# OSUrobotics/KinovaGrasping

Measured on AMD Instinct MI355X. Metric: env-steps/sec (whole node) at 4096 envs/GPU, higher is better.
Workload: dtype f32

## Files before the change

### kinovagrasping_amd/csrc/ks_api.hip

```cpp
#include <hip/hip_runtime.h>

#include <algorithm>
#include <cstdio>
#include <cstdlib>
#include <cstring>
#include <type_traits>
#include <map>
#include <string>
#include <vector>

#include "../../include/kinova_sim.h"
#include "ks_env.h"
#include "ks_mlp_tile.h"
#include "ks_select.h"
#include "ks_model_host.h"

using namespace ks;

namespace {

constexpr int WAVE = 64;
thread_local std::string g_create_error;

template <typename T> struct StartPool {
// ... 699 lines not shown
    const long bi = (long)sel * N + i;
    const long len0 = ra.with_replay ? ra.cur_len[bi] : 0;
    const long tt = len0 < H - 1 ? len0 : H - 1;
    const long row = bi * H + tt;
    for (int c = sub; c < S; c += SUBS) {
        const float so = (float)((const R*)ra.sim_obs)[(long)i * S + c];
        const float st = ra.obs[(long)i * S + c];
        const float nx = done ? (float)((const R*)ra.sim_final_obs)[(long)i * S + c] : so;
        if (store) { ra.cur_state[row * S + c] = st; ra.cur_next[row * S + c] = nx; }
        ra.prev_obs[(long)i * S + c] = done ? so : st;
        ra.obs[(long)i * S + c] = so;
    }
    if (store && sub < A) ra.cur_action[row * A + sub] = ra.action[(long)i * A + sub];
    if (sub != 0) return;
    long len1 = len0;
    if (store) {
        ra.cur_reward[row] = rew;
        ra.cur_not_done[row] = done ? 0.0f : 1.0f;
        len1 = tt + 1;
    }
    if (ra.with_replay) {
        if (done && lift && len1 > 0) {
            ra.cur_reward[bi * H + len1 - 1] = rew;
            ra.cur_not_done[bi * H + len1 - 1] = 0.0f;
        }
        ra.cur_len[bi] = len1;
        if (done) {
            const bool keep = len1 - ra.n_steps > 1;
            const long bo = (long)(sel ^ 1) * N + i;
            const bool free_other = __hip_atomic_load(&ra.pub_len[bo], __ATOMIC_ACQUIRE, __HIP_MEMORY_SCOPE_AGENT) == 0;
#ifdef KS_DEBUG_DROPS
            int64_t* dbg = ra.counters + 8 + 4 * 512 + 8;
            if (keep && !free_other) {
                const long long gap = (long long)ra.steps_total[i] - (long long)dbg[i];
                atomicAdd((unsigned long long*)&ra.counters[4], (unsigned long long)gap);
                atomicAdd((unsigned long long*)&ra.counters[5], 1ull);
                atomicMin((long long*)&ra.counters[6], gap);
                __builtin_amdgcn_fence(__ATOMIC_ACQUIRE, "agent");
                if (__hip_atomic_load(&ra.pub_len[bo], __ATOMIC_ACQUIRE, __HIP_MEMORY_SCOPE_AGENT) == 0) atomicAdd((unsigned long long*)&ra.counters[7], 1ull);
            }
            if (keep && free_other) dbg[i] = ra.steps_total[i];
#endif
            if (keep && free_other) {
                __threadfence();
                __hip_atomic_store(&ra.pub_len[bi], (int64_t)len1, __ATOMIC_RELEASE, __HIP_MEMORY_SCOPE_AGENT);
                ra.cur_sel[i] = (uint8_t)(sel ^ 1);
                ra.cur_len[bo] = 0;
                atomicAdd((unsigned long long*)&ra.counters[2], 1ull);
            } else {
                ra.cur_len[bi] = 0;
                if (keep) atomicAdd((unsigned long long*)&ra.counters[3], 1ull);
            }
        }
    }
    if (done) {
        atomicAdd((unsigned long long*)&ra.counters[0], 1ull);
        if (ra.sim_done[i] & 1) atomicAdd((unsigned long long*)&ra.counters[1], 1ull);
    }
    ra.has_prev[i] = !done;
    ra.t[i] = done ? 0 : ra.t[i] + 1;
    __hip_atomic_store(&ra.steps_total[i], ra.steps_total[i] + 1, __ATOMIC_RELAXED, __HIP_MEMORY_SCOPE_AGENT);
    ra.ready[i] = (ra.ready[i] != 0) && !done;
    ra.reward_out[i] = rew;
    ra.done_out[i] = done;
}

constexpr int ROLLOUT_QCAP = 2048, ROLLOUT_Q_STEPS = 16, ROLLOUT_Q_RING = ROLLOUT_Q_STEPS + ROLLOUT_QCAP, ROLLOUT_Q_WORDS = ROLLOUT_Q_RING + ROLLOUT_QCAP;
__global__ void k_rollout_queue_init(int* __restrict__ queue, int n_groups) {
    for (int i = threadIdx.x; i < ROLLOUT_Q_WORDS; i += blockDim.x) {
        int v = 0;
        if (i == 1) v = n_groups;
        if (i >= ROLLOUT_Q_RING && i - ROLLOUT_Q_RING < n_groups) v = (1 << 12) | (i - ROLLOUT_Q_RING + 1);
        queue[i] = v;
    }
}

template <int NT1, int NT2>
__device__ __noinline__ void rollout_policy_wave(const ks_rollout_args* __restrict__ rap, int N, int row_env, KS_LDS float* wblocks) {
    const ks_rollout_args& ra = *rap;
    const int S = krsel::S, A = krsel::A;
    constexpr int NR = 4;
    kmlp::f32x4(*H1)[NR] = (kmlp::f32x4(*)[NR])(float*)wblocks;
    kmlp::f32x4(*H2)[NR] = H1 + NT1 * 4;
    const int lane = threadIdx.x & 63;
    for (;;) {
        const long long ver = uniform64(__hip_atomic_load(ra.actor_ver, __ATOMIC_RELAXED, __HIP_MEMORY_SCOPE_AGENT));
        __builtin_amdgcn_fence(__ATOMIC_ACQUIRE, "agent");
        const float* pw = ra.actor_pub + (ver % 3) * ra.actor_stride;
        kmlp::f32x4 z4 = {0.f, 0.f, 0.f, 0.f};
        const bool mine = kmlp::mlp3_rows_wave<NT1, NT2, true, NR>(lane, (long)row_env, S, ra.h1, ra.h2, A, ra.obs, S, kmlp::x_bytes(N, 0, S, S), pw + ra.off_w1,
                                                                     pw + ra.off_b1, pw + ra.off_w2, pw + ra.off_b2, pw + ra.off_w3, H1, H2, z4);
        float y[4] = {0.f, 0.f, 0.f, 0.f};
        if (mine) policy_squash(ra, z4, pw + ra.off_b3, y);
        __builtin_amdgcn_fence(__ATOMIC_ACQUIRE, "agent");
        const long long ver2 = uniform64(__hip_atomic_load(ra.actor_ver, __ATOMIC_RELAXED, __HIP_MEMORY_SCOPE_AGENT));
        if (ver2 - ver < 2) {
            if (mine) policy_select(ra, N, row_env, y);
            return;
        }
        if (lane == 0 && ra.repeats) atomicAdd((unsigned long long*)ra.repeats, 1ull);
    }
}

#ifdef KS_ROLLOUT_STAMP
#define KS_RS(i) { const long long t1_ = wall_clock64(); if (C::tid() == 0) atomicAdd((unsigned long long*)&rap->counters[4 + i], (unsigned long long)(t1_ - tk)); tk = t1_; }
#else
#define KS_RS(i)
#endif
template <int NT1, int NT2, bool WAVE_SCOPE>
__device__ __forceinline__ void rollout_iter(const Model<float>& m, const Hulls<float>& hu, const Buffers<float>* __restrict__ bdev, int N, int frame_skip,
                                             int iters, int epw, int pair_memory, const ObsOut<float>* __restrict__ out,
                                             const ks_rollout_args* __restrict__ rap, KS_LDS float* blocks, int grp) {
    using T = float;
    using C = Crew<WAVE_SCOPE>;
    const Buffers<T>& b = *bdev;
    const int e = threadIdx.x / LANE_STRIDE;
    const Team<SUBS> team{(int)threadIdx.x % LANE_STRIDE};
    const int env = e < epw ? b.slot_env[grp * epw + e] : -1;
    const bool active = !(team.sub >= SUBS || env < 0);
    const int wave = WAVE_SCOPE ? (int)(threadIdx.x >> 6) : 0;
    const int slot0 = grp * epw + 4 * wave, cepw = WAVE_SCOPE ? (epw - 4 * wave < 4 ? (epw - 4 * wave < 0 ? 0 : epw - 4 * wave) : 4) : epw;
    KS_LDS T* cblocks = blocks + 4 * wave * SCR_TOTAL;
    KS_LDS unsigned* w = (KS_LDS unsigned*)cblocks;
    const auto join = [] {
        if constexpr (!WAVE_SCOPE) __threadfence_block();
        C::sync();
    };
#ifdef KS_ROLLOUT_STAMP
    long long tk = wall_clock64();
#endif
    {
        const int nn = C::tid() & 15;
        const int row_env = nn < cepw ? b.slot_env[slot0 + nn] : -1;
        if (b.ctl->mode != 0) rollout_controller(b.ctl, rap, N, C::tid() < 16 ? row_env : -1);
        else if constexpr (WAVE_SCOPE) rollout_policy_wave<NT1, NT2>(rap, N, row_env, cblocks);
        else rollout_policy<NT1, NT2>(rap, N, row_env, cblocks);
    }
    join();
    KS_RS(0)
    if (active) {
        T hq[4], act[4];
        KS_UNROLL
        for (int i = 0; i < 4; i++) { hq[i] = b.hand_quat[(long)i * N + env]; act[i] = rap->action_t[(long)i * N + env]; }
        int ncon = 0, status = 0;
        ColW<T> snap{b.snap + env, N};
        KS_LDS T* blk = blocks + e * SCR_TOTAL;
        ScratchC<T, KS_LDS T*> scr{blk};
        T* stp = (T*)(blk + SCR_STATE);
        load_state_team<T, SUBS>(b, env, N, stp, team.sub);
        load_env_params(scr, team, b, env, N);
        constexpr int WPL = (NPAIR_MAX + SUBS - 1) / SUBS;
        PairWarm gw[WPL];
        unsigned* pm = b.pairmem + ((long)env * SUBS + team.sub) * (WPL * WARM_WORDS);
        KS_UNROLL
        for (int q = 0; q < WPL; q++) {
            KS_UNROLL
            for (int j = 0; j < WARM_WORDS; j++) gw[q].w[j] = pair_memory ? pm[q * WARM_WORDS + j] : 0u;
        }
        lane_env_step(m, hu, *(LaneState<T>*)stp, hq, act, scr, team, snap, frame_skip, iters, ncon, status, (float*)nullptr, stp + NQ + 2 * NV, gw,
                      []() {});
        if (pair_memory) {
            KS_UNROLL
            for (int q = 0; q < WPL; q++) {
                KS_UNROLL
                for (int j = 0; j < WARM_WORDS; j++) pm[q * WARM_WORDS + j] = gw[q].w[j];
            }
        }
        team.sync();
        store_state_team<T, SUBS>(b, env, N, stp, team.sub);
        if (status) atomicOr(&b.status[env], status);
        if (team.sub == 0) b.ncon[env] = ncon;
    }
    join();
    KS_RS(1)
// ... 1034 lines not shown
    }
    void reset_pass(const Buffers<T>& e, void* obs, hipStream_t s) {
        const int N = cfg.n_envs;
        hipLaunchKernelGGL((k_reset<T, USE_LDS>), dim3(blocks()), dim3(WAVE), 0, s, d_model, e, N, 0);
        hipLaunchKernelGGL((k_rays<T>), dim3((N + RAY_ENVS - 1) / RAY_ENVS, NRAY), dim3(WAVE), 0, s, d_model, e, N, 1);
        hipLaunchKernelGGL((k_obs<T>), dim3(blocks()), dim3(WAVE), 0, s, d_model, e, N, 1, out_record(obs, nullptr, nullptr, nullptr, nullptr));
    }
    int post_reset(void* obs, hipStream_t s) {
        if (b.rayq) HIPCHK(hipMemsetAsync(b.rayq, 0, (4 + 2 * (size_t)n_wg) * sizeof(int32_t), s));
        reset_pass(b, obs, s);
        HIPCHK(hipGetLastError());
        return KS_OK;
    }
    int reset(const int32_t* ids, int n, const void* q0, const void* hq, const int32_t* object_id, const void* mass_friction, void* obs,
              hipStream_t s) override {
        if (int r = need_model("ks_reset")) return r;
        if (n <= 0 || n > cfg.n_envs || !q0 || !hq || (!ids && n != cfg.n_envs)) { error = "ks_reset: bad arguments"; return KS_ERR_INVALID; }
        hipLaunchKernelGGL((k_store_init<T>), dim3((n + 255) / 256), dim3(256), 0, s, b, ids, n, (const T*)q0, (const T*)hq, object_id,
                           (const T*)mass_friction, n_models, cfg.n_envs);
        if (object_id) {
            clear_pool(s);
            clear_ranges(s);
            if (n_models > 1)
                if (int r = regroup(s)) return r;
        }
        return post_reset(obs, s);
    }
    int step(const void* action, void* obs, void* reward, uint8_t* done, void* info, void* final_obs, hipStream_t s) override {
        if (int r = need_model("ks_step")) return r;
        if (!action) { error = "ks_step: action is NULL"; return KS_ERR_INVALID; }
        const int N = cfg.n_envs;
        const bool timed = ev_used < NEV && (step_calls++ % ev_stride) == 0;
        const ObsOut<T> out = out_record(obs, reward, done, info, final_obs);
        const bool capturing = stream_is_capturing(s);
        if (obs_in_step && (capturing || captured_out > 0 || !(out == out_sent && out_valid))) {
            out_valid = !capturing;
            out_sent = out;
            ObsOut<T>* slot = pinned_record(capturing, h_out, (unsigned)h_out_next++, captured_out);
            if (!slot) { error = "ks_step: more captured calls than the context keeps output records for"; return KS_ERR_STATE; }
            *slot = out;
            HIPCHK(hipMemcpyAsync(d_out, slot, sizeof out, hipMemcpyHostToDevice, s));
        }
        if (timed) HIPCHK(hipEventRecord(ev0[ev_used], s));
        hipLaunchKernelGGL(step_kernel(), dim3(n_wg), dim3(WG), step_lds, s, d_model, b, (const Buffers<T>*)d_b, (const T*)action, N, cfg.frame_skip,
                           cfg.solver_iterations, lpw, cfg.contact_tap, (int)rays_in_step, (int)(USE_LDS && cfg.pair_memory), (int)obs_in_step,
                           (const ObsOut<T>*)d_out, ray_pool, n_wg);
        if (timed) { HIPCHK(hipEventRecord(ev1[ev_used], s)); ev_used++; }
        if (!rays_in_step) hipLaunchKernelGGL((k_rays<T>), dim3((N + RAY_ENVS - 1) / RAY_ENVS, NRAY), dim3(WAVE), 0, s, d_model, b, N, 0);
        if (!obs_in_step) hipLaunchKernelGGL((k_obs<T>), dim3(blocks()), dim3(WAVE), 0, s, d_model, b, N, 0, out);
        HIPCHK(hipGetLastError());
        return KS_OK;
    }
    int check_rollout_buffers(int n_iter, const ks_rollout_args* ra) {
        if (!ra || n_iter <= 0 || (ctl_mode == 0 && (!ra->actor_pub || !ra->actor_ver)) || !ra->obs || !ra->prev_obs || !ra->has_prev || !ra->ready || !ra->lifting ||
            !ra->t || !ra->steps_total || !ra->action || !ra->action_t || !ra->reward_out || !ra->done_out || !ra->sim_obs || !ra->sim_reward ||
            !ra->sim_done || !ra->sim_info || !ra->sim_final_obs || !ra->counters) { error = "ks_rollout: NULL argument"; return KS_ERR_INVALID; }
        if (ra->with_replay && (!ra->cur_state || !ra->cur_next || !ra->cur_action || !ra->cur_reward || !ra->cur_not_done || !ra->cur_len ||
                                !ra->cur_sel || !ra->pub_len || ra->horizon <= ra->n_steps)) { error = "ks_rollout: replay buffers"; return KS_ERR_INVALID; }
        return KS_OK;
    }
    int check_rollout_actor(const ks_rollout_args* ra) {
        if (ctl_mode != 0) return KS_OK;
        if ((ra->off_w2 | ra->off_w3 | ra->actor_stride) & 3) { error = "ks_rollout: weight offsets must be multiples of 4 floats"; return KS_ERR_INVALID; }
        if ((ra->h1 | ra->h2) & 3) { error = "ks_rollout: hidden widths must be multiples of 4"; return KS_ERR_INVALID; }
        if ((int64_t)cfg.n_envs * krsel::S * 4 >= (int64_t)kmlp::OOR) { error = "ks_rollout: the observation rows exceed the actor's 32-bit lane offsets"; return KS_ERR_INVALID; }
        return KS_OK;
    }
    int send_rollout_records(const ks_rollout_args* ra, hipStream_t s) {
        const ObsOut<T> out = out_record(ra->sim_obs, ra->sim_reward, ra->sim_done, ra->sim_info, ra->sim_final_obs);
        const bool capturing = stream_is_capturing(s);
        ObsOut<T>* slot = pinned_record(capturing, h_out, (unsigned)h_out_next++, captured_out);
        if (!slot) { error = "ks_rollout: more captured calls than the context keeps output records for"; return KS_ERR_STATE; }
        *slot = out;
        out_valid = false;
        HIPCHK(hipMemcpyAsync(d_out, slot, sizeof out, hipMemcpyHostToDevice, s));
        ks_rollout_args* rslot = pinned_record(capturing, h_ra, h_ra_next++, captured_ra);
        if (!rslot) { error = "ks_rollout: more captured calls than the context keeps argument records for"; return KS_ERR_STATE; }
        *rslot = *ra;
        HIPCHK(hipMemcpyAsync(d_ra, rslot, sizeof *ra, hipMemcpyHostToDevice, s));
        return KS_OK;
    }
    static constexpr int policy_tiles(int h1, int h2) { return (h1 + 15) / 16 + (h2 + 15) / 16; }
    static constexpr size_t policy_lds_bytes(int h1, int h2) { return (size_t)(policy_tiles(h1, h2) * 4 + 4) * 16 * 16 + 16; }
    static constexpr size_t policy_wave_lds_bytes(int h1, int h2) { return (size_t)(policy_tiles(h1, h2) * 4) * 4 * 16; }
    template <int A, int B> struct Tiles { static constexpr int NT1 = A, NT2 = B; };
    template <typename F> int launch_for_widths(const ks_rollout_args* ra, F launch) {
        const int t1 = (ra->h1 + 15) / 16, t2 = (ra->h2 + 15) / 16;
        if (t1 == 16 && t2 == 16) return launch(Tiles<16, 16>{});
        if (t1 == 25 && t2 == 19) return launch(Tiles<25, 19>{});
        if (t1 == 8 && t2 == 8) return launch(Tiles<8, 8>{});
        if (t1 == 4 && t2 == 4) return launch(Tiles<4, 4>{});
        if (ctl_mode != 0) return launch(Tiles<16, 16>{});
        error = "ks_rollout: hidden widths must be 256-256, 400-300, 128-128 or 64-64";
        return KS_ERR_INVALID;
    }
    template <typename K, typename... A> int launch_rollout(K kernel, size_t lds, hipStream_t s, A... args) {
        HIPCHK(hipFuncSetAttribute((const void*)kernel, hipFuncAttributeMaxDynamicSharedMemorySize, (int)lds));
        hipLaunchKernelGGL(kernel, dim3(n_groups < resident_wgs ? n_groups : resident_wgs), dim3(WG), lds, s, args...);
        HIPCHK(hipGetLastError());
        return KS_OK;
    }
    int rollout_exact(int n_iter, const ks_rollout_args* ra, hipStream_t s) {
#ifdef KS_MULTI_GEOM
        (void)n_iter; (void)ra; (void)s;
        error = "ks_rollout: libkinova_sim_mg.so runs fp32 contexts only (the exact mode, precision 64, is in libkinova_sim.so)";
        return KS_ERR_INVALID;
#else
        int r;
        if ((r = check_rollout_buffers(n_iter, ra))) return r;
        if (!cfg.obs_env_major || !cfg.auto_reset) { error = "ks_rollout needs env-major observations and auto_reset"; return KS_ERR_STATE; }
        if ((r = check_rollout_actor(ra))) return r;
        if (ra->budget_ticks != 0) { error = "ks_rollout: a time budget needs the wave form of the rollout kernel (ks_rollout_plan: KS_PLAN_WAVES); fp64 contexts have none"; return KS_ERR_STATE; }
        const size_t ws_offset = (step_lds + 15) / 16 * 16;
        const size_t lds = ws_offset + std::max(policy_lds_bytes(ra->h1, ra->h2), (size_t)F64_RAY_BYTES);
        if (lds > 160 * 1024) { error = "ks_rollout: no LDS for the policy beside this object's hull tables"; return KS_ERR_STATE; }
        if ((r = send_rollout_records(ra, s))) return r;
        return launch_for_widths(ra, [&](auto tiles) {
            using W = decltype(tiles);
            return launch_rollout(k_rollout_f64<W::NT1, W::NT2>, lds, s, d_model, b, (const Buffers<T>*)d_b, cfg.n_envs, cfg.frame_skip, cfg.solver_iterations,
                                  lpw, (const ObsOut<T>*)d_out, (const ks_rollout_args*)d_ra, n_iter, rollout_round_robin ? -n_groups : n_groups,
                                  (int)ws_offset);
        });
#endif
    }
    int rollout(int n_iter, const ks_rollout_args* ra, hipStream_t s) override {
        if (int r = need_model("ks_rollout")) return r;
        if constexpr (sizeof(T) != 4) return rollout_exact(n_iter, ra, s);
        else {
            int r;
            if ((r = check_rollout_buffers(n_iter, ra))) return r;
            if (!obs_in_step || !cfg.obs_env_major || !cfg.auto_reset) { error = "ks_rollout needs the in-kernel observation path, env-major observations and auto_reset"; return KS_ERR_STATE; }
            if ((r = check_rollout_actor(ra))) return r;
            if (policy_lds_bytes(ra->h1, ra->h2) > (size_t)SCR_TOTAL * lpw * sizeof(T)) { error = "ks_rollout: no LDS for the policy"; return KS_ERR_STATE; }
            const int N = cfg.n_envs;
            const bool wave_free = plan_waves() && policy_wave_lds_bytes(ra->h1, ra->h2) <= (size_t)SCR_TOTAL * 4 * sizeof(T);
            if (ra->budget_ticks != 0 && (ra->budget_ticks < 0 || !wave_free)) {
                error = "ks_rollout: a time budget needs the wave form of the rollout kernel (ks_rollout_plan: KS_PLAN_WAVES)";
                return KS_ERR_STATE;
            }
            if ((r = send_rollout_records(ra, s))) return r;
            const bool use_queue = plan_queue();
            if (use_queue) {
                hipLaunchKernelGGL(k_rollout_queue_init, dim3(1), dim3(256), 0, s, d_queue, n_groups);
            }
            if (wave_free && rollout_phase_deal != 0 && n_models == 1 && ra->budget_ticks == 0) {
                if (rollout_phase_deal == 2 && N <= PHASE_ENVS_MAX) hipLaunchKernelGGL(k_slots_by_phase, dim3(1), dim3(PHASE_THREADS), 0, s, (const int64_t*)ra->t, N, n_wg * lpw, b.slot_env);
                else if (lpw <= 16) hipLaunchKernelGGL(k_slots_by_phase_in_groups, dim3((n_groups + 255) / 256), dim3(256), 0, s, (const int64_t*)ra->t, n_groups, lpw, b.slot_env);
            }
            return launch_for_widths(ra, [&](auto tiles) {
                using W = decltype(tiles);
                return launch_rollout(k_rollout<W::NT1, W::NT2>, step_lds, s, d_model, b, (const Buffers<T>*)d_b, N, cfg.frame_skip, cfg.solver_iterations, lpw,
                                      (int)cfg.pair_memory, (const ObsOut<T>*)d_out, (const ks_rollout_args*)d_ra, n_iter,
                                      (use_queue || !rollout_round_robin) ? n_groups : -n_groups, use_queue ? d_queue : (int*)nullptr, (int)wave_free);
            });
        }
    }
    bool plan_queue() const { return rollout_queue && n_groups > resident_wgs && n_groups <= ROLLOUT_QCAP; }
    bool plan_waves() const {
        return rollout_waves && !plan_queue() && n_groups <= resident_wgs && lpw == EPW_MAX && LANE_STRIDE == SUBS &&
               (size_t)(wg_rays_words(4, WAVE) + wg_obs_words(4) + 4) <= (size_t)SCR_TOTAL * 4;
    }
    int rollout_plan(int32_t* mode, int32_t* groups, int32_t* workgroups) override {
        if (int r = need_model("ks_rollout_plan")) return r;
        if constexpr (sizeof(T) != 4) {
            if (mode) *mode = n_groups <= resident_wgs ? KS_PLAN_WORKGROUPS : (rollout_round_robin ? KS_PLAN_ROUND_ROBIN : KS_PLAN_RUNS);
        } else if (mode) *mode = plan_waves() ? KS_PLAN_WAVES : (n_groups <= resident_wgs ? KS_PLAN_WORKGROUPS : (plan_queue() ? KS_PLAN_QUEUE : (rollout_round_robin ? KS_PLAN_ROUND_ROBIN : KS_PLAN_RUNS)));
        if (groups) *groups = n_groups;
// ... 331 lines not shown
```

### kinovagrasping_amd/csrc/ks_mlp_tile.h

```cpp
#pragma once
#include <stdint.h>

#if defined(__HIPCC__)
#include <hip/hip_runtime.h>
#define KS_MLP_HD __host__ __device__
#else
#define KS_MLP_HD
#endif

namespace kmlp {

constexpr int ROWS = 16;
constexpr int KS_IN_MAX = 6;

constexpr uint32_t OOR = 0x7ffffff0u;

KS_MLP_HD inline uint32_t tile_soff(int row0, int k0, int K) { return (uint32_t)(row0 * K + k0) * 4u; }
KS_MLP_HD inline uint32_t quad_off(int nn, int q, int row0, int nrow, int k0, int K) {
    const int row = row0 + nn, k = k0 + 4 * q;
    return (row >= 0 && row < nrow && k + 3 < K) ? (uint32_t)(nn * K + 4 * q) * 4u : OOR;
}
KS_MLP_HD inline int tail_k(int K) { return K & ~3; }
KS_MLP_HD inline uint32_t tail_off(int nn, int row0, int nrow, int K, int j) {
    const int row = row0 + nn;
// ... 113 lines not shown
                    const float fb = ldf(rXb, x_off(row, 16 * s + 4 * q + j, in_a, in_dim, ldb), 0);
                    fa[s][j] = 16 * s + 4 * q + j < in_a ? fa[s][j] : fb;
                }
        }
#pragma unroll
        for (int s = 0; s < KS_IN_MAX; s++) bx[s] = f32x4{fa[s][0], fa[s][1], fa[s][2], fa[s][3]};
    }
    Tile<NT1, !VEC> a2, b2t;
    {
        Tile<KS_IN_MAX, true> a1, b1t;
        a1.issue(rW1, rB1, nn, q, 16 * wave, h1, in_dim);
        a2.issue(rW2, rB2, nn, q, 16 * wave, h2, h1);
        auto tile1 = [&](const Tile<KS_IN_MAX, true>& w, int t) {
            f32x4 acc0 = {0.f, 0.f, 0.f, 0.f}, acc1 = {0.f, 0.f, 0.f, 0.f};
#pragma unroll
            for (int s = 0; s < KS_IN_MAX; s++) {
                if (s & 1) acc1 = mfma4(w.quad(s, q, in_dim), bx[s], acc1);
                else acc0 = mfma4(w.quad(s, q, in_dim), bx[s], acc0);
            }
            const f32x4 hq = bias_relu(acc0 + acc1, w.bias(q, 16 * t, h1), t * 16 + 4 * q, h1);
            H1[t * 4 + q][nn] = hq;
            if (h1_out && row_ok && t * 16 + 4 * q < h1) *(f32x4*)(h1_out + (long)row * h1 + t * 16 + 4 * q) = hq;
        };
#pragma unroll 1
        for (int t = wave; t < NT1; t += 2 * NW) {
            if (NT1 > NW) b1t.issue(rW1, rB1, nn, q, 16 * (t + NW), h1, in_dim);
            tile1(a1, t);
            if (NT1 > 2 * NW) a1.issue(rW1, rB1, nn, q, 16 * (t + 2 * NW), h1, in_dim);
            if (NT1 > NW && t + NW < NT1) tile1(b1t, t + NW);
        }
    }
    __syncthreads();

    constexpr int NJ = (NT2 + NW - 1) / NW;
    f32x4 w3[NJ];
    float w3t[3];
#pragma unroll
    for (int j = 0; j < NJ; j++) w3[j] = ldq(rW3, quad_off(nn, q, 0, out_dim, 16 * (wave + NW * j), h2), tile_soff(0, 16 * (wave + NW * j), h2));
    if (!VEC) {
#pragma unroll
        for (int j = 0; j < 3; j++) w3t[j] = ldf(rW3, tail_off(nn, 0, out_dim, h2, j), 0);
    }
    __builtin_amdgcn_sched_barrier(0);
    auto tile2 = [&](const Tile<NT1, !VEC>& w, int t) {
        f32x4 acc0 = {0.f, 0.f, 0.f, 0.f}, acc1 = {0.f, 0.f, 0.f, 0.f};
#pragma unroll
        for (int s = 0; s < NT1; s++) {
            if (s & 1) acc1 = mfma4(w.quad(s, q, h1), H1[s * 4 + q][nn], acc1);
            else acc0 = mfma4(w.quad(s, q, h1), H1[s * 4 + q][nn], acc0);
        }
        const f32x4 hq = bias_relu(acc0 + acc1, w.bias(q, 16 * t, h2), t * 16 + 4 * q, h2);
        H2[t * 4 + q][nn] = hq;
        if (h2_out && row_ok && t * 16 + 4 * q < h2) *(f32x4*)(h2_out + (long)row * h2 + t * 16 + 4 * q) = hq;
    };
#pragma unroll 1
    for (int t = wave; t < NT2; t += 2 * NW) {
        if (NT2 > NW) b2t.issue(rW2, rB2, nn, q, 16 * (t + NW), h2, h1);
        tile2(a2, t);
        if (NT2 > 2 * NW) a2.issue(rW2, rB2, nn, q, 16 * (t + 2 * NW), h2, h1);
        if (NT2 > NW && t + NW < NT2) tile2(b2t, t + NW);
    }
    __syncthreads();

    {
        f32x4 acc = {0.f, 0.f, 0.f, 0.f};
#pragma unroll
        for (int j = 0; j < NJ; j++)
            if (wave + NW * j < NT2) {
                const f32x4 wq = (!VEC && tail_here(q, 16 * (wave + NW * j), h2)) ? f32x4{w3t[0], w3t[1], w3t[2], 0.f} : w3[j];
                acc = mfma4(wq, H2[(wave + NW * j) * 4 + q][nn], acc);
            }
        if (q == 0) P[wave][nn] = acc;
    }
    __syncthreads();
    if (wave == 0 && q == 0 && row_ok) {
        z4 = P[0][nn];
#pragma unroll
        for (int w = 1; w < NW; w++) z4 += P[w][nn];
        return true;
    }
    return false;
}

template <int NT1, int NT2, bool VEC, int NR>
__device__ __forceinline__ bool mlp3_rows_wave(const int lane, const long row, int in_dim, int h1, int h2, int out_dim, const float* __restrict__ xa, int lda,
                                               uint32_t xa_bytes, const float* __restrict__ W1, const float* __restrict__ b1,
                                               const float* __restrict__ W2, const float* __restrict__ b2, const float* __restrict__ W3,
                                               f32x4 (*H1)[NR], f32x4 (*H2)[NR], f32x4& z4) {
    const int nn = lane & 15, q = lane >> 4;
    const bool row_ok = row >= 0, col_ok = nn < NR;
    const f32x4 zero = {0.f, 0.f, 0.f, 0.f};
    in_dim = uni(in_dim), h1 = uni(h1), h2 = uni(h2), out_dim = uni(out_dim), lda = uni(lda);
    const rsrc_t rW1 = rsrc(W1, (uint32_t)(h1 * in_dim) * 4u), rB1 = rsrc(b1, (uint32_t)h1 * 4u), rW2 = rsrc(W2, (uint32_t)(h2 * h1) * 4u),
                 rB2 = rsrc(b2, (uint32_t)h2 * 4u), rW3 = rsrc(W3, (uint32_t)(out_dim * h2) * 4u);
    f32x4 bx[KS_IN_MAX];
    {
        const rsrc_t rXa = rsrc(xa, xa_bytes);
#pragma unroll
        for (int s = 0; s < KS_IN_MAX; s++) {
            float v[4];
#pragma unroll
            for (int j = 0; j < 4; j++) v[j] = ldf(rXa, x_off(row, 16 * s + 4 * q + j, 0, in_dim, lda), 0);
            bx[s] = f32x4{v[0], v[1], v[2], v[3]};
        }
    }
    Tile<NT1, !VEC> a2, b2t;
    {
        Tile<KS_IN_MAX, true> a1, b1t;
        a1.issue(rW1, rB1, nn, q, 0, h1, in_dim);
        a2.issue(rW2, rB2, nn, q, 0, h2, h1);
        auto tile1 = [&](const Tile<KS_IN_MAX, true>& w, int t) {
            f32x4 acc0 = zero, acc1 = zero;
#pragma unroll
            for (int s = 0; s < KS_IN_MAX; s++) {
                if (s & 1) acc1 = mfma4(w.quad(s, q, in_dim), bx[s], acc1);
                else acc0 = mfma4(w.quad(s, q, in_dim), bx[s], acc0);
            }
            const f32x4 hq = bias_relu(acc0 + acc1, w.bias(q, 16 * t, h1), t * 16 + 4 * q, h1);
            if (col_ok) H1[t * 4 + q][nn] = hq;
        };
#pragma unroll 1
        for (int t = 0; t < NT1; t += 2) {
            b1t.issue(rW1, rB1, nn, q, 16 * (t + 1), h1, in_dim);
            tile1(a1, t);
            a1.issue(rW1, rB1, nn, q, 16 * (t + 2), h1, in_dim);
            if (t + 1 < NT1) tile1(b1t, t + 1);
        }
    }
    __builtin_amdgcn_fence(__ATOMIC_RELEASE, "wavefront");
    __builtin_amdgcn_wave_barrier();
    __builtin_amdgcn_fence(__ATOMIC_ACQUIRE, "wavefront");

    constexpr bool HOLD_B = NT1 <= 16;
    f32x4 hb[HOLD_B ? NT1 : 1];
    if (HOLD_B) {
#pragma unroll
        for (int s = 0; s < NT1; s++) hb[s] = col_ok ? H1[s * 4 + q][nn] : zero;
    }
    auto tile2 = [&](const Tile<NT1, !VEC>& w, int t) {
        f32x4 acc0 = zero, acc1 = zero;
#pragma unroll
        for (int s = 0; s < NT1; s++) {
            const f32x4 b = HOLD_B ? hb[HOLD_B ? s : 0] : (col_ok ? H1[s * 4 + q][nn] : zero);
            if (s & 1) acc1 = mfma4(w.quad(s, q, h1), b, acc1);
            else acc0 = mfma4(w.quad(s, q, h1), b, acc0);
        }
        const f32x4 hq = bias_relu(acc0 + acc1, w.bias(q, 16 * t, h2), t * 16 + 4 * q, h2);
        if (col_ok) H2[t * 4 + q][nn] = hq;
    };
#pragma unroll 1
    for (int t = 0; t < NT2; t += 2) {
        b2t.issue(rW2, rB2, nn, q, 16 * (t + 1), h2, h1);
        tile2(a2, t);
        a2.issue(rW2, rB2, nn, q, 16 * (t + 2), h2, h1);
        if (t + 1 < NT2) tile2(b2t, t + 1);
    }
    f32x4 w3[NT2];
    float w3t[3];
#pragma unroll
    for (int s = 0; s < NT2; s++) w3[s] = ldq(rW3, quad_off(nn, q, 0, out_dim, 16 * s, h2), tile_soff(0, 16 * s, h2));
    if (!VEC) {
#pragma unroll
        for (int j = 0; j < 3; j++) w3t[j] = ldf(rW3, tail_off(nn, 0, out_dim, h2, j), 0);
    }
    __builtin_amdgcn_sched_barrier(0);
    __builtin_amdgcn_fence(__ATOMIC_RELEASE, "wavefront");
    __builtin_amdgcn_wave_barrier();
    __builtin_amdgcn_fence(__ATOMIC_ACQUIRE, "wavefront");

    f32x4 part[NW];
#pragma unroll
    for (int w = 0; w < NW; w++) {
        f32x4 acc = zero;
#pragma unroll
        for (int j = 0; j < (NT2 + NW - 1) / NW; j++)
            if (w + NW * j < NT2) {
                const int s = w + NW * j;
                const f32x4 wq = (!VEC && tail_here(q, 16 * s, h2)) ? f32x4{w3t[0], w3t[1], w3t[2], 0.f} : w3[s];
                acc = mfma4(wq, col_ok ? H2[s * 4 + q][nn] : zero, acc);
            }
        part[w] = acc;
    }
    if (q == 0 && row_ok && col_ok) {
        z4 = part[0];
#pragma unroll
        for (int w = 1; w < NW; w++) z4 += part[w];
        return true;
    }
    return false;
}

}
#endif
```

Measured before the change: 2.907 million.

## Rewrite wave-scoped policy MLP with 4x4x1 MFMA row blocks

Replaces the 16-row mfma4 tiling in the per-wave policy MLP with 4x4x1 f32 MFMAs that put four batch rows in one block. Each lane now loads a whole weight row quad, and weights are double-buffered in register sets across k-steps and layers. Observations are staged into a new LDS region (X), and the layer-3 partial sums are reduced with lane shuffles instead of held per wave. This targets the MFMA work and weight-load traffic that the 16-row tiles spent when only a few rows (NR=4) are live, at the cost of more MFMA instructions, a larger wave LDS footprint and register pressure.

```diff
diff --git a/kinovagrasping_amd/csrc/ks_api.hip b/kinovagrasping_amd/csrc/ks_api.hip
--- a/kinovagrasping_amd/csrc/ks_api.hip
+++ b/kinovagrasping_amd/csrc/ks_api.hip
@@ -805,14 +805,17 @@
     constexpr int NR = 4;
     kmlp::f32x4(*H1)[NR] = (kmlp::f32x4(*)[NR])(float*)wblocks;
     kmlp::f32x4(*H2)[NR] = H1 + NT1 * 4;
+    kmlp::f32x4(*X)[NR] = H2 + NT2 * 4;
     const int lane = threadIdx.x & 63;
     for (;;) {
         const long long ver = uniform64(__hip_atomic_load(ra.actor_ver, __ATOMIC_RELAXED, __HIP_MEMORY_SCOPE_AGENT));
         __builtin_amdgcn_fence(__ATOMIC_ACQUIRE, "agent");
         const float* pw = ra.actor_pub + (ver % 3) * ra.actor_stride;
         kmlp::f32x4 z4 = {0.f, 0.f, 0.f, 0.f};
-        const bool mine = kmlp::mlp3_rows_wave<NT1, NT2, true, NR>(lane, (long)row_env, S, ra.h1, ra.h2, A, ra.obs, S, kmlp::x_bytes(N, 0, S, S), pw + ra.off_w1,
-                                                                     pw + ra.off_b1, pw + ra.off_w2, pw + ra.off_b2, pw + ra.off_w3, H1, H2, z4);
+        int ln = lane, rw = row_env;
+        asm volatile("" : "+v"(ln), "+v"(rw));
+        const bool mine = kmlp::mlp3_rows_wave<NT1, NT2, true, NR>(ln, (long)rw, S, ra.h1, ra.h2, A, ra.obs, S, kmlp::x_bytes(N, 0, S, S), pw + ra.off_w1,
+                                                                     pw + ra.off_b1, pw + ra.off_w2, pw + ra.off_b2, pw + ra.off_w3, X, H1, H2, z4);
         float y[4] = {0.f, 0.f, 0.f, 0.f};
         if (mine) policy_squash(ra, z4, pw + ra.off_b3, y);
         __builtin_amdgcn_fence(__ATOMIC_ACQUIRE, "agent");
@@ -2013,7 +2016,7 @@
     }
     static constexpr int policy_tiles(int h1, int h2) { return (h1 + 15) / 16 + (h2 + 15) / 16; }
     static constexpr size_t policy_lds_bytes(int h1, int h2) { return (size_t)(policy_tiles(h1, h2) * 4 + 4) * 16 * 16 + 16; }
-    static constexpr size_t policy_wave_lds_bytes(int h1, int h2) { return (size_t)(policy_tiles(h1, h2) * 4) * 4 * 16; }
+    static constexpr size_t policy_wave_lds_bytes(int h1, int h2) { return (size_t)(policy_tiles(h1, h2) * 4 + kmlp::KS_IN_MAX * 4) * 4 * 16; }
     template <int A, int B> struct Tiles { static constexpr int NT1 = A, NT2 = B; };
     template <typename F> int launch_for_widths(const ks_rollout_args* ra, F launch) {
         const int t1 = (ra->h1 + 15) / 16, t2 = (ra->h2 + 15) / 16;
diff --git a/kinovagrasping_amd/csrc/ks_mlp_tile.h b/kinovagrasping_amd/csrc/ks_mlp_tile.h
--- a/kinovagrasping_amd/csrc/ks_mlp_tile.h
+++ b/kinovagrasping_amd/csrc/ks_mlp_tile.h
@@ -219,109 +219,190 @@
     return false;
 }
 
+__device__ __forceinline__ f32x4 mfma1(float a, float b, f32x4 c) { return __builtin_amdgcn_mfma_f32_4x4x1f32(a, b, c, 0, 0, 0); }
+
+struct Rows4Set {
+    f32x4 w[16];
+};
+
+template <int G>
+__device__ __forceinline__ void rows4_issue(Rows4Set& t, rsrc_t rW, int lane, int row0, int nrow, int s, int K) {
+    __builtin_amdgcn_sched_barrier(0);
+#pragma unroll
+    for (int g = 0; g < G; g++)
+#pragma unroll
+        for (int q = 0; q < 4; q++) t.w[4 * g + q] = ldq(rW, quad_off(lane, q, row0 + 64 * g, nrow, 16 * s, K), tile_soff(row0 + 64 * g, 16 * s, K));
+    __builtin_amdgcn_sched_barrier(0);
+}
+template <int G>
+__device__ __forceinline__ void rows4_tails(float* wt, rsrc_t rW, int lane, int row0, int nrow, int K) {
+#pragma unroll
+    for (int g = 0; g < G; g++)
+#pragma unroll
+        for (int j = 0; j < 3; j++) wt[3 * g + j] = ldf(rW, tail_off(lane, row0 + 64 * g, nrow, K, j), tile_soff(row0 + 64 * g, 0, K));
+    __builtin_amdgcn_sched_barrier(0);
+}
+
+template <int G, bool TAIL, int NR>
+__device__ __forceinline__ void rows4_kstep(const Rows4Set& t, const float* wt, f32x4 (&acc)[G], const f32x4 (*Bsrc)[NR], int lane, int s, int K) {
+    const f32x4 zero = {0.f, 0.f, 0.f, 0.f};
+    const bool col_ok = (lane & 3) < NR;
+    f32x4 b[4], a[G][4];
+#pragma unroll
+    for (int q = 0; q < 4; q++) {
+        b[q] = col_ok ? Bsrc[4 * s + q][col_ok ? lane & 3 : 0] : zero;
+#pragma unroll
+        for (int g = 0; g < G; g++)
+            a[g][q] = (TAIL && tail_here(q, 16 * s, K)) ? f32x4{wt[3 * g], wt[3 * g + 1], wt[3 * g + 2], 0.f} : t.w[4 * g + q];
+    }
+#pragma unroll
+    for (int x = 0; x < 4; x++)
+#pragma unroll
+        for (int q = 0; q < 4; q++)
+#pragma unroll
+            for (int g = 0; g < G; g++) acc[g] = mfma1(a[g][q][x], b[q][x], acc[g]);
+}
+
+template <int G, int NP, int NS, bool TAILW, bool TAILB, int NR, int NQ, class FA, class FB>
+__device__ __forceinline__ void rows4_layer(rsrc_t rW, rsrc_t rB, int lane, int nfeat, int K, const f32x4 (*Bsrc)[NR], f32x4 (*Hout)[NR], Rows4Set& a,
+                                            Rows4Set& b, float* wt, FA next_a, FB next_b) {
+    constexpr int NSE = (NS + 1) & ~1;
+    const f32x4 zero = {0.f, 0.f, 0.f, 0.f};
+    const int fq = lane >> 2;
+#pragma unroll
+    for (int p = 0; p < NP; p++) {
+        const int o0 = 64 * G * p;
+        f32x4 acc0[G], acc1[G];
+#pragma unroll
+        for (int g = 0; g < G; g++) acc0[g] = acc1[g] = zero;
+#pragma unroll 1
+        for (int s = 0; s + 2 < NSE; s += 2) {
+            rows4_kstep<G, TAILW, NR>(a, wt, acc0, Bsrc, lane, s, K);
+            rows4_issue<G>(a, rW, lane, o0, nfeat, s + 2, K);
+            rows4_kstep<G, TAILW, NR>(b, wt, acc1, Bsrc, lane, s + 1, K);
+            rows4_issue<G>(b, rW, lane, o0, nfeat, s + 3, K);
+        }
+        f32x4 bq[G];
+        float bt[3];
+#pragma unroll
+        for (int g = 0; g < G; g++) bq[g] = ldq(rB, quad_off(0, fq, 0, 1, o0 + 64 * g, nfeat), tile_soff(0, o0 + 64 * g, nfeat));
+        if (TAILB) {
+#pragma unroll
+            for (int j = 0; j < 3; j++) bt[j] = ldf(rB, tail_off(0, 0, 1, nfeat, j), 0);
+        }
+        __builtin_amdgcn_sched_barrier(0);
+        rows4_kstep<G, TAILW, NR>(a, wt, acc0, Bsrc, lane, NSE - 2, K);
+        if (p + 1 < NP) rows4_issue<G>(a, rW, lane, o0 + 64 * G, nfeat, 0, K);
+        else next_a();
+        if (NSE - 1 < NS) rows4_kstep<G, TAILW, NR>(b, wt, acc1, Bsrc, lane, NSE - 1, K);
+        if (p + 1 < NP) {
+            rows4_issue<G>(b, rW, lane, o0 + 64 * G, nfeat, 1, K);
+            if (TAILW) rows4_tails<G>(wt, rW, lane, o0 + 64 * G, nfeat, K);
+        } else next_b();
+#pragma unroll
+        for (int g = 0; g < G; g++) {
+            const int f = o0 + 64 * g + 4 * fq;
+            const f32x4 bias = (TAILB && tail_here(fq, o0 + 64 * g, nfeat)) ? f32x4{bt[0], bt[1], bt[2], 0.f} : bq[g];
+            const f32x4 hq = bias_relu(acc0[g] + acc1[g], bias, f, nfeat);
+            if ((lane & 3) < NR && (f >> 2) < NQ) Hout[f >> 2][lane & 3] = hq;
+        }
+    }
+}
+
+__device__ __forceinline__ void rows4_join() {
+    __builtin_amdgcn_fence(__ATOMIC_RELEASE, "wavefront");
+    __builtin_amdgcn_wave_barrier();
+    __builtin_amdgcn_fence(__ATOMIC_ACQUIRE, "wavefront");
+}
+
+constexpr int rows4_passes(int NT) { return ((NT + 3) / 4 + 3) / 4; }
+constexpr int rows4_groups(int NT) { return ((NT + 3) / 4 + rows4_passes(NT) - 1) / rows4_passes(NT); }
+
 template <int NT1, int NT2, bool VEC, int NR>
 __device__ __forceinline__ bool mlp3_rows_wave(const int lane, const long row, int in_dim, int h1, int h2, int out_dim, const float* __restrict__ xa, int lda,
                                                uint32_t xa_bytes, const float* __restrict__ W1, const float* __restrict__ b1,
                                                const float* __restrict__ W2, const float* __restrict__ b2, const float* __restrict__ W3,
-                                               f32x4 (*H1)[NR], f32x4 (*H2)[NR], f32x4& z4) {
-    const int nn = lane & 15, q = lane >> 4;
-    const bool row_ok = row >= 0, col_ok = nn < NR;
+                                               f32x4 (*X)[NR], f32x4 (*H1)[NR], f32x4 (*H2)[NR], f32x4& z4) {
+    static_assert(NR >= 1 && NR <= 4, "one MFMA block holds four batch rows");
+    constexpr int G1 = rows4_groups(NT1), NP1 = rows4_passes(NT1), G2 = rows4_groups(NT2), NP2 = rows4_passes(NT2);
+    constexpr int NJ = (NT2 + NW - 1) / NW, NQ3 = 4 * NJ;
+    static_assert(NQ3 <= 32, "layer 3's quads fill at most the two register sets");
     const f32x4 zero = {0.f, 0.f, 0.f, 0.f};
     in_dim = uni(in_dim), h1 = uni(h1), h2 = uni(h2), out_dim = uni(out_dim), lda = uni(lda);
     const rsrc_t rW1 = rsrc(W1, (uint32_t)(h1 * in_dim) * 4u), rB1 = rsrc(b1, (uint32_t)h1 * 4u), rW2 = rsrc(W2, (uint32_t)(h2 * h1) * 4u),
                  rB2 = rsrc(b2, (uint32_t)h2 * 4u), rW3 = rsrc(W3, (uint32_t)(out_dim * h2) * 4u);
-    f32x4 bx[KS_IN_MAX];
+    constexpr int XW = 16 * KS_IN_MAX, XN = (NR * XW + 63) / 64;
+    float xv[XN];
     {
         const rsrc_t rXa = rsrc(xa, xa_bytes);
 #pragma unroll
-        for (int s = 0; s < KS_IN_MAX; s++) {
-            float v[4];
-#pragma unroll
-            for (int j = 0; j < 4; j++) v[j] = ldf(rXa, x_off(row, 16 * s + 4 * q + j, 0, in_dim, lda), 0);
-            bx[s] = f32x4{v[0], v[1], v[2], v[3]};
-        }
-    }
-    Tile<NT1, !VEC> a2, b2t;
-    {
-        Tile<KS_IN_MAX, true> a1, b1t;
-        a1.issue(rW1, rB1, nn, q, 0, h1, in_dim);
-        a2.issue(rW2, rB2, nn, q, 0, h2, h1);
-        auto tile1 = [&](const Tile<KS_IN_MAX, true>& w, int t) {
-            f32x4 acc0 = zero, acc1 = zero;
-#pragma unroll
-            for (int s = 0; s < KS_IN_MAX; s++) {
-                if (s & 1) acc1 = mfma4(w.quad(s, q, in_dim), bx[s], acc1);
-                else acc0 = mfma4(w.quad(s, q, in_dim), bx[s], acc0);
-            }
-            const f32x4 hq = bias_relu(acc0 + acc1, w.bias(q, 16 * t, h1), t * 16 + 4 * q, h1);
-            if (col_ok) H1[t * 4 + q][nn] = hq;
-        };
-#pragma unroll 1
-        for (int t = 0; t < NT1; t += 2) {
-            b1t.issue(rW1, rB1, nn, q, 16 * (t + 1), h1, in_dim);
-            tile1(a1, t);
-            a1.issue(rW1, rB1, nn, q, 16 * (t + 2), h1, in_dim);
-            if (t + 1 < NT1) tile1(b1t, t + 1);
-        }
-    }
-    __builtin_amdgcn_fence(__ATOMIC_RELEASE, "wavefront");
-    __builtin_amdgcn_wave_barrier();
-    __builtin_amdgcn_fence(__ATOMIC_ACQUIRE, "wavefront");
-
-    constexpr bool HOLD_B = NT1 <= 16;
-    f32x4 hb[HOLD_B ? NT1 : 1];
-    if (HOLD_B) {
-#pragma unroll
-        for (int s = 0; s < NT1; s++) hb[s] = col_ok ? H1[s * 4 + q][nn] : zero;
-    }
-    auto tile2 = [&](const Tile<NT1, !VEC>& w, int t) {
-        f32x4 acc0 = zero, acc1 = zero;
-#pragma unroll
-        for (int s = 0; s < NT1; s++) {
-            const f32x4 b = HOLD_B ? hb[HOLD_B ? s : 0] : (col_ok ? H1[s * 4 + q][nn] : zero);
-            if (s & 1) acc1 = mfma4(w.quad(s, q, h1), b, acc1);
-            else acc0 = mfma4(w.quad(s, q, h1), b, acc0);
-        }
-        const f32x4 hq = bias_relu(acc0 + acc1, w.bias(q, 16 * t, h2), t * 16 + 4 * q, h2);
-        if (col_ok) H2[t * 4 + q][nn] = hq;
+        for (int j = 0; j < XN; j++) {
+            const int i = lane + 64 * j, r = i / XW;
+            const int rowr = __shfl((int)row, r < NR ? r : 0);
+            xv[j] = ldf(rXa, x_off(r < NR ? (long)rowr : -1L, i % XW, 0, in_dim, lda), 0);
+        }
+    }
+    Rows4Set a, b;
+    float wt[12], wt3[3];
+    rows4_issue<G1>(a, rW1, lane, 0, h1, 0, in_dim);
+    rows4_issue<G1>(b, rW1, lane, 0, h1, 1, in_dim);
+    rows4_tails<G1>(wt, rW1, lane, 0, h1, in_dim);
+#pragma unroll
+    for (int j = 0; j < XN; j++) {
+        const int i = lane + 64 * j, r = i / XW, k = i % XW;
+        if (r < NR) ((float*)X)[((k >> 2) * NR + r) * 4 + (k & 3)] = xv[j];
+    }
+    rows4_join();
+    rows4_layer<G1, NP1, KS_IN_MAX, true, !VEC, NR, NT1 * 4>(
+        rW1, rB1, lane, h1, in_dim, X, H1, a, b, wt, [&] { rows4_issue<G2>(a, rW2, lane, 0, h2, 0, h1); },
+        [&] {
+            rows4_issue<G2>(b, rW2, lane, 0, h2, 1, h1);
+            if (!VEC) rows4_tails<G2>(wt, rW2, lane, 0, h2, h1);
+        });
+    rows4_join();
+
+    const int w3 = lane >> 2, r3 = w3 < NW ? lane & 3 : -1;
+    const auto issue3 = [&](Rows4Set& t, int i0) {
+        __builtin_amdgcn_sched_barrier(0);
+#pragma unroll
+        for (int i = i0; i < NQ3 && i < i0 + 16; i++) t.w[i - i0] = ldq(rW3, quad_off(r3, 4 * (w3 + NW * (i >> 2)) + (i & 3), 0, out_dim, 0, h2), 0);
+        if (!VEC && i0 == 0) {
+#pragma unroll
+            for (int j = 0; j < 3; j++) wt3[j] = ldf(rW3, tail_off(r3, 0, out_dim, h2, j), 0);
+        }
+        __builtin_amdgcn_sched_barrier(0);
     };
-#pragma unroll 1
-    for (int t = 0; t < NT2; t += 2) {
-        b2t.issue(rW2, rB2, nn, q, 16 * (t + 1), h2, h1);
-        tile2(a2, t);
-        a2.issue(rW2, rB2, nn, q, 16 * (t + 2), h2, h1);
-        if (t + 1 < NT2) tile2(b2t, t + 1);
-    }
-    f32x4 w3[NT2];
-    float w3t[3];
-#pragma unroll
-    for (int s = 0; s < NT2; s++) w3[s] = ldq(rW3, quad_off(nn, q, 0, out_dim, 16 * s, h2), tile_soff(0, 16 * s, h2));
-    if (!VEC) {
-#pragma unroll
-        for (int j = 0; j < 3; j++) w3t[j] = ldf(rW3, tail_off(nn, 0, out_dim, h2, j), 0);
-    }
-    __builtin_amdgcn_sched_barrier(0);
-    __builtin_amdgcn_fence(__ATOMIC_RELEASE, "wavefront");
-    __builtin_amdgcn_wave_barrier();
-    __builtin_amdgcn_fence(__ATOMIC_ACQUIRE, "wavefront");
-
-    f32x4 part[NW];
-#pragma unroll
-    for (int w = 0; w < NW; w++) {
-        f32x4 acc = zero;
-#pragma unroll
-        for (int j = 0; j < (NT2 + NW - 1) / NW; j++)
-            if (w + NW * j < NT2) {
-                const int s = w + NW * j;
-                const f32x4 wq = (!VEC && tail_here(q, 16 * s, h2)) ? f32x4{w3t[0], w3t[1], w3t[2], 0.f} : w3[s];
-                acc = mfma4(wq, col_ok ? H2[s * 4 + q][nn] : zero, acc);
-            }
-        part[w] = acc;
-    }
-    if (q == 0 && row_ok && col_ok) {
-        z4 = part[0];
-#pragma unroll
-        for (int w = 1; w < NW; w++) z4 += part[w];
+    rows4_layer<G2, NP2, NT1, !VEC, !VEC, NR, NT2 * 4>(rW2, rB2, lane, h2, h1, H1, H2, a, b, wt, [&] { issue3(a, 0); }, [&] { issue3(b, 16); });
+    rows4_join();
+
+    f32x4 acc = zero;
+    const bool col_ok = (lane & 3) < NR;
+#pragma unroll
+    for (int j = 0; j < NJ; j++) {
+        const int s = w3 + NW * j;
+        const bool ok = w3 < NW && s < NT2;
+        f32x4 hq[4], wq[4], n = acc;
+#pragma unroll
+        for (int q = 0; q < 4; q++) {
+            hq[q] = (ok && col_ok) ? H2[(ok ? s : 0) * 4 + q][col_ok ? lane & 3 : 0] : zero;
+            const int i = 4 * j + q;
+            wq[q] = i < 16 ? a.w[i < 16 ? i : 0] : b.w[i < 16 ? 0 : i - 16];
+            if (!VEC) wq[q] = tail_here(4 * s + q, 0, h2) ? f32x4{wt3[0], wt3[1], wt3[2], 0.f} : wq[q];
+        }
+#pragma unroll
+        for (int x = 0; x < 4; x++)
+#pragma unroll
+            for (int q = 0; q < 4; q++) n = mfma1(wq[q][x], hq[q][x], n);
+        acc = (NT2 % NW == 0 || j + 1 < NJ || ok) ? n : acc;
+    }
+    f32x4 z = acc;
+#pragma unroll
+    for (int w = 1; w < NW; w++) {
+        const int src = 4 * w + (lane & 3);
+        z += f32x4{__shfl(acc.x, src), __shfl(acc.y, src), __shfl(acc.z, src), __shfl(acc.w, src)};
+    }
+    if (lane < NR && row >= 0) {
+        z4 = z;
         return true;
     }
     return false;
```

Result: faster. 2.938 million, median of 6 (+1.1%).
